# mindazhao/PWStableNet

Measured on AMD Instinct MI355X. Metric: stabilized frames/sec at 256x256 (netG fp32 + grid_sample), whole job, higher is better.
Workload: dtype f32

## Files before the change

### pwstablenet_amd/csrc/conv_common.h

```cpp
#pragma once
#include "common.h"

namespace pws {

typedef float f32x16 __attribute__((ext_vector_type(16)));

struct ConvKParams {
    const float *src_ptr[4];
    int src_c[4];
    int src_ld[4];
    int nsrc;
    int N, H, W;
    int LH, LW;
    int OH, OW;
    int cin_pad;
    int cout;
    const float *w;
    const float *bias;
    float *out;
    int out_ld;
    int act;
    int tiles_x, tiles_y;
    unsigned ntiles;
    int nclasses;
    int cls_inner;
    int ksplit;
    int chunks_per_split;
    size_t split_stride;
    const void *w_bf;
    int kpad_bf, npad_bf;
    int io_bf16;
    int epi16;
    int ndst;
    float *dst_ptr[4];
    int dst_c0[4], dst_c1[4], dst_ld[4], dst_acc[4];
    const void *dst_y[4];
    int dst_y_ld[4], dst_act[4];
    void *out_sign;
    int out_sign_ld;
    const void *dst_sign[4];
    int dst_sign_ld[4];
};

__device__ __forceinline__ void epi_store(const ConvKParams &p, size_t pix, int co, float v) {
    if (p.ndst == 0) {
        p.out[pix * p.out_ld + co] = act_apply(v + (p.bias ? p.bias[co] : 0.f), p.act);
    } else {
#pragma unroll
        for (int s = 0; s < 4; ++s) {
            if (s < p.ndst && co >= p.dst_c0[s] && co < p.dst_c1[s]) {
                float *d = p.dst_ptr[s] + pix * p.dst_ld[s] + (co - p.dst_c0[s]);
                *d = p.dst_acc[s] ? *d + v : v;
            }
        }
    }
}

__device__ __forceinline__ float bf16_lo(unsigned u) { return __builtin_bit_cast(float, u << 16); }
__device__ __forceinline__ float bf16_hi(unsigned u) { return __builtin_bit_cast(float, u & 0xffff0000u); }
__device__ __forceinline__ void epi_store_pair16(const ConvKParams &p, size_t pix, int co, float v0, float v1) {
    if (p.ndst == 0) {
        const float b0 = p.bias ? p.bias[co] : 0.f, b1 = p.bias ? p.bias[co + 1] : 0.f;
        unsigned *d = reinterpret_cast<unsigned *>(reinterpret_cast<__bf16 *>(p.out) + pix * p.out_ld + co);
        *d = cvt_pk_bf16(act_apply(v0 + b0, p.act), act_apply(v1 + b1, p.act));
    } else {
#pragma unroll
        for (int s = 0; s < 4; ++s) {
            if (s < p.ndst && co >= p.dst_c0[s] && co < p.dst_c1[s]) {
                unsigned *d = reinterpret_cast<unsigned *>(reinterpret_cast<__bf16 *>(p.dst_ptr[s]) + pix * p.dst_ld[s] + (co - p.dst_c0[s]));
                if (p.dst_acc[s]) {
                    const unsigned o = *d;
                    v0 += bf16_lo(o), v1 += bf16_hi(o);
                }
                if (p.dst_act[s] != PWS_ACT_NONE) {
                    const unsigned y = *reinterpret_cast<const unsigned *>(static_cast<const __bf16 *>(p.dst_y[s]) + pix * p.dst_y_ld[s] +
                                                                           (co - p.dst_c0[s]));
                    const float sl = p.dst_act[s] == PWS_ACT_LRELU ? 0.2f : 0.f;
                    v0 *= bf16_lo(y) > 0.f ? 1.f : sl, v1 *= bf16_hi(y) > 0.f ? 1.f : sl;
                }
                *d = cvt_pk_bf16(v0, v1);
            }
        }
    }
}

__device__ __forceinline__ void conv_block_coords(const ConvKParams &p, bool subpix, unsigned &tile, int &cls, int &split) {
    if (subpix && p.cls_inner) {
        const unsigned xcd = blockIdx.x & 7u, slot = blockIdx.x >> 3;
        cls = (int)(slot & 3u), split = (int)blockIdx.z;
        tile = xcd_remap(((slot >> 2) << 3) | xcd, p.ntiles);
    } else {
        tile = xcd_remap(blockIdx.x, p.ntiles);
        cls = subpix ? (int)(blockIdx.z & 3) : 0;
        split = subpix ? (int)(blockIdx.z >> 2) : (int)blockIdx.z;
    }
}
static inline dim3 conv_grid(ConvKParams &kp, int bn) {
    kp.cls_inner = kp.nclasses == 4 && kp.ntiles % 8 == 0 ? 1 : 0;
    const unsigned gy = (unsigned)((kp.cout + bn - 1) / bn);
    return kp.cls_inner ? dim3(kp.ntiles * 4, gy, (unsigned)kp.ksplit) : dim3(kp.ntiles, gy, (unsigned)(kp.nclasses * kp.ksplit));
}

struct ProfInfo {
    double flops, bytes;
};

struct TileChoice {
    int th, tw, tn, ck, bn;
    int kid;
    int (*launch)(ConvKParams &, hipStream_t, const ProfInfo &);
};

int launch_splitk_reduce(const ConvKParams &kp, const float *partial, size_t total4, hipStream_t st);

static inline long cdiv(long a, long b) { return (a + b - 1) / b; }

constexpr long kFillBlocks = 512;
constexpr long kFillBlocksBf16 = 256;

[[maybe_unused]] static int select_and_launch(const TileChoice *cands, int ncand, ConvKParams &kp, int cin_total, float *final_out,
                             float *ws, size_t ws_floats, hipStream_t st, const ProfInfo &pi, long kFill = kFillBlocks) {
    const TileChoice *best = nullptr;
    long best_blocks = -1;
    double best_score = -1.0;
// ... 42 lines not shown
```

### pwstablenet_amd/csrc/conv_mfma.hip

```cpp
#include "conv_common.h"

namespace pws {

template <int KS_, int STRIDE_, int PAD_, int SUBPIX_, int TH_, int TW_, int TN_, int CK_, int WM_, int WN_, int MT_,
          int NT_, bool NCHW_ = false>
struct ConvCfg {
    static constexpr int KS = KS_, STRIDE = STRIDE_, PAD = PAD_, TH = TH_, TW = TW_, TN = TN_, CK = CK_;
    static constexpr int SUBPIX = SUBPIX_;
    static constexpr bool CONVT = SUBPIX_ != 0, NCHW = NCHW_;
    static constexpr int WM = WM_, WN = WN_, MT = MT_, NT = NT_;
    static constexpr int THREADS = 64 * WM * WN;
    static constexpr int BM = TH * TW * TN, BN = 32 * NT * WN;
    static_assert(BM == 32 * MT * WM, "tile pixels must equal the M extent of the wave grid");
    static constexpr int IH = (TH - 1) * STRIDE + KS, IW = (TW - 1) * STRIDE + KS;
    static constexpr int PIX = TN * IH * IW;
    static constexpr int CKP = CK + 1;
    static constexpr int TAPS = KS * KS;
    static constexpr int LDS_IN = (PIX * CKP + 3) / 4 * 4;
    static constexpr int LDS_W = TAPS * CK * BN;
    static constexpr int LDS_BYTES = (LDS_IN + LDS_W) * 4;
    static constexpr int C4 = CK / 4;
    static constexpr int ITEMS_IN = (PIX * C4 + THREADS - 1) / THREADS;
    static constexpr int ITEMS_W = (TAPS * CK * (BN / 4) + THREADS - 1) / THREADS;
    static constexpr int ITEMS_NCHW = (PIX * CK + THREADS - 1) / THREADS;
};

template <class C>
__global__ void __launch_bounds__(C::THREADS, 2) conv_mfma_kernel(const ConvKParams p) {
    extern __shared__ float lds[];
    float *lds_in = lds;
    float *lds_w = lds + C::LDS_IN;

    const int tid = threadIdx.x;
    const int lane = tid & 63, wv = tid >> 6;
    const int l31 = lane & 31, hi = lane >> 5;
    const int wm = wv / C::WN, wn = wv % C::WN;

    unsigned tile;
    int cls, split;
    conv_block_coords(p, C::CONVT, tile, cls, split);
    const int tx_i = tile % p.tiles_x;
    const int ty_i = (tile / p.tiles_x) % p.tiles_y;
    const int tn_i = tile / (p.tiles_x * p.tiles_y);
    const int n0 = tn_i * C::TN, y0 = ty_i * C::TH, x0 = tx_i * C::TW;
    const int co0 = blockIdx.y * C::BN;
    const int py = cls >> 1, px = cls & 1;
    const int pad_y = C::SUBPIX == 1 ? 1 - py : (C::SUBPIX == 2 ? 0 : C::PAD);
    const int pad_x = C::SUBPIX == 1 ? 1 - px : (C::SUBPIX == 2 ? 0 : C::PAD);
    const int iy0 = y0 * C::STRIDE - pad_y, ix0 = x0 * C::STRIDE - pad_x;

    int g_pix[C::ITEMS_IN];
    int l_off[C::ITEMS_IN];
    int g_c4[C::ITEMS_IN];
    unsigned ok_mask = 0;
#pragma unroll
    for (int it = 0; it < C::ITEMS_IN; ++it) {
        const int item = tid + it * C::THREADS;
        const int pix = item / C::C4, c4 = item % C::C4;
        const int lx = pix % C::IW, ly = (pix / C::IW) % C::IH, tn = pix / (C::IW * C::IH);
        const int n = n0 + tn, iy = iy0 + ly, ix = ix0 + lx;
        const bool ok = item < C::PIX * C::C4 && n < p.N && iy >= 0 && iy < p.H && ix >= 0 && ix < p.W;
        g_pix[it] = ok ? (n * p.H + iy) * p.W + ix : 0;
        ok_mask |= ok ? (1u << it) : 0u;
        l_off[it] = item < C::PIX * C::C4 ? pix * C::CKP + c4 * 4 : -1;
        g_c4[it] = c4 * 4;
    }
    static_assert(C::ITEMS_IN <= 32 && C::ITEMS_W <= 32, "mask width");
    int w_off[C::ITEMS_W];
    unsigned w_mask = 0;
#pragma unroll
    for (int it = 0; it < C::ITEMS_W; ++it) {
        const int item = tid + it * C::THREADS;
        const int row = item / (C::BN / 4), q = item % (C::BN / 4);
        const int tap = row / C::CK, c = row % C::CK;
        const bool ok = item < C::TAPS * C::CK * (C::BN / 4) && (co0 + q * 4) < p.cout;
        w_off[it] = ok ? (tap * p.cin_pad + c) * p.cout + co0 + q * 4 : 0;
        w_mask |= ok ? (1u << it) : 0u;
    }
    const float *w_cls = p.w + (size_t)cls * C::TAPS * p.cin_pad * p.cout;
    float4 r_in[C::NCHW ? 1 : C::ITEMS_IN];
    float4 r_w[C::ITEMS_W];
    float r_nchw[C::NCHW ? C::ITEMS_NCHW : 1];

    auto load_chunk = [&](int s, int c0, int wrow) {
        if constexpr (C::NCHW) {
            const int Creal = p.src_c[0];
            const size_t sstride = p.src_ld[0] ? (size_t)p.src_ld[0] : (size_t)Creal * p.H * p.W;
#pragma unroll
            for (int it = 0; it < C::ITEMS_NCHW; ++it) {
                const int item = tid + it * C::THREADS;
                const int c = item / C::PIX, pix = item % C::PIX;
                const int lx = pix % C::IW, ly = (pix / C::IW) % C::IH, tn = pix / (C::IW * C::IH);
                const int n = n0 + tn, iy = iy0 + ly, ix = ix0 + lx;
                const bool ok = item < C::PIX * C::CK && (c0 + c) < Creal && n < p.N && iy >= 0 && iy < p.H && ix >= 0 &&
                                ix < p.W;
                const size_t off = ok ? (size_t)n * sstride + ((size_t)(c0 + c) * p.H + iy) * p.W + ix : 0;
                const float v = p.src_ptr[0][off];
                r_nchw[it] = ok ? v : 0.f;
            }
        } else {
            const float *sp = p.src_ptr[s] + c0;
            const size_t ld = p.src_ld[s];
#pragma unroll
            for (int it = 0; it < C::ITEMS_IN; ++it)
                r_in[it] = *reinterpret_cast<const float4 *>(sp + (size_t)g_pix[it] * ld + g_c4[it]);
        }
        const float *wp = w_cls + (size_t)wrow * p.cout;
#pragma unroll
        for (int it = 0; it < C::ITEMS_W; ++it) r_w[it] = *reinterpret_cast<const float4 *>(wp + w_off[it]);
    };
    auto store_chunk = [&]() {
        if constexpr (C::NCHW) {
#pragma unroll
            for (int it = 0; it < C::ITEMS_NCHW; ++it) {
                const int item = tid + it * C::THREADS;
                const int c = item / C::PIX, pix = item % C::PIX;
                if (item < C::PIX * C::CK) lds_in[pix * C::CKP + c] = r_nchw[it];
            }
        } else {
#pragma unroll
            for (int it = 0; it < C::ITEMS_IN; ++it) {
                if (l_off[it] >= 0) {
                    const bool ok = (ok_mask >> it) & 1u;
                    float *d = lds_in + l_off[it];
                    d[0] = ok ? r_in[it].x : 0.f, d[1] = ok ? r_in[it].y : 0.f, d[2] = ok ? r_in[it].z : 0.f,
                    d[3] = ok ? r_in[it].w : 0.f;
                }
            }
        }
#pragma unroll
        for (int it = 0; it < C::ITEMS_W; ++it) {
            const int item = tid + it * C::THREADS;
            if (item < C::TAPS * C::CK * (C::BN / 4)) {
                const bool ok = (w_mask >> it) & 1u;
                *reinterpret_cast<float4 *>(lds_w + item * 4) =
                    ok ? r_w[it] : make_float4(0.f, 0.f, 0.f, 0.f);
            }
        }
    };

    f32x16 acc[C::MT][C::NT];
#pragma unroll
    for (int mt = 0; mt < C::MT; ++mt)
#pragma unroll
        for (int nt = 0; nt < C::NT; ++nt)
#pragma unroll
            for (int r = 0; r < 16; ++r) acc[mt][nt][r] = 0.f;

    int a_base[C::MT];
#pragma unroll
    for (int mt = 0; mt < C::MT; ++mt) {
        const int m = (wm * C::MT + mt) * 32 + l31;
        const int tx = m % C::TW, ty = (m / C::TW) % C::TH, tn = m / (C::TW * C::TH);
        a_base[mt] = ((tn * C::IH + ty * C::STRIDE) * C::IW + tx * C::STRIDE) * C::CKP + hi;
    }
    const int b_base = hi * C::BN + wn * C::NT * 32 + l31;

    int total_chunks = 0;
    if constexpr (C::NCHW) {
        total_chunks = p.cin_pad / C::CK;
    } else {
        for (int s = 0; s < p.nsrc; ++s) total_chunks += p.src_c[s] / C::CK;
    }
    const int ch_begin = split * p.chunks_per_split;
    const int ch_end = min(total_chunks, ch_begin + p.chunks_per_split);
    int s = 0, c0 = ch_begin * C::CK, wrow = ch_begin * C::CK;
    if constexpr (!C::NCHW) {
        while (s < p.nsrc - 1 && c0 >= p.src_c[s]) c0 -= p.src_c[s], ++s;
    }
    if (ch_begin < ch_end) load_chunk(s, c0, wrow);
    for (int ch = ch_begin; ch < ch_end; ++ch) {
        __syncthreads();
        store_chunk();
        __syncthreads();
        c0 += C::CK, wrow += C::CK;
        if (!C::NCHW && c0 >= p.src_c[s]) ++s, c0 = 0;
        if (ch + 1 < ch_end) load_chunk(s, c0, wrow);

#pragma unroll
        for (int tap = 0; tap < C::TAPS; ++tap) {
            if (C::SUBPIX == 2 && ((!py && tap / C::KS) || (!px && tap % C::KS))) continue;
            const int toff = ((tap / C::KS) * C::IW + (tap % C::KS)) * C::CKP;
#pragma unroll
            for (int kk = 0; kk < C::CK / 2; ++kk) {
                float a[C::MT], b[C::NT];
#pragma unroll
                for (int mt = 0; mt < C::MT; ++mt) a[mt] = lds_in[a_base[mt] + toff + 2 * kk];
#pragma unroll
                for (int nt = 0; nt < C::NT; ++nt) b[nt] = lds_w[b_base + (tap * C::CK + 2 * kk) * C::BN + nt * 32];
#pragma unroll
                for (int mt = 0; mt < C::MT; ++mt)
#pragma unroll
                    for (int nt = 0; nt < C::NT; ++nt)
                        acc[mt][nt] = __builtin_amdgcn_mfma_f32_32x32x2f32(a[mt], b[nt], acc[mt][nt], 0, 0, 0);
            }
        }
    }

    const bool partial = p.ksplit > 1;
    float *part = p.out + (size_t)split * p.split_stride;
#pragma unroll
    for (int nt = 0; nt < C::NT; ++nt) {
        const int co = co0 + (wn * C::NT + nt) * 32 + l31;
        const bool co_ok = co < p.cout;
#pragma unroll
        for (int mt = 0; mt < C::MT; ++mt) {
#pragma unroll
            for (int r = 0; r < 16; ++r) {
                const int m = (wm * C::MT + mt) * 32 + (r & 3) + 8 * (r >> 2) + 4 * hi;
                const int tx = m % C::TW, ty = (m / C::TW) % C::TH, tn = m / (C::TW * C::TH);
                const int n = n0 + tn, y = y0 + ty, x = x0 + tx;
                const int oy = C::CONVT ? 2 * y + py : y, ox = C::CONVT ? 2 * x + px : x;
                if (co_ok && n < p.N && y < p.LH && x < p.LW && oy < p.OH && ox < p.OW) {
                    const size_t pix = (size_t)(n * p.OH + oy) * p.OW + ox;
                    if (partial)
                        part[pix * p.cout + co] = acc[mt][nt][r];
                    else
                        epi_store(p, pix, co, acc[mt][nt][r]);
                }
            }
        }
    }
}

__global__ void __launch_bounds__(256) splitk_reduce_kernel(const ConvKParams p, const float *__restrict__ partial,
                                                            size_t total4) {
    const size_t i = (size_t)blockIdx.x * 256 + threadIdx.x;
    if (i >= total4) return;
    float4 a = reinterpret_cast<const float4 *>(partial)[i];
    for (int s = 1; s < p.ksplit; ++s) {
        const float4 b = reinterpret_cast<const float4 *>(partial + (size_t)s * p.split_stride)[i];
        a.x += b.x, a.y += b.y, a.z += b.z, a.w += b.w;
    }
    const size_t pix = (i * 4) / p.cout;
    const int co = (int)((i * 4) % p.cout);
    if (p.io_bf16) {
        epi_store_pair16(p, pix, co, a.x, a.y), epi_store_pair16(p, pix, co + 2, a.z, a.w);
        return;
    }
    epi_store(p, pix, co, a.x), epi_store(p, pix, co + 1, a.y), epi_store(p, pix, co + 2, a.z), epi_store(p, pix, co + 3, a.w);
}

int launch_splitk_reduce(const ConvKParams &kp, const float *partial, size_t total4, hipStream_t st) {
    hipLaunchKernelGGL(splitk_reduce_kernel, dim3((unsigned)((total4 + 255) / 256)), dim3(256), 0, st, kp, partial, total4);
    return check_launch("splitk_reduce_kernel");
}

template <class C, int KID>
static int launch_cfg(ConvKParams &kp, hipStream_t st, const ProfInfo &pi) {
    static PerDeviceFlag attr_set_dev;
    bool &attr_set = attr_set_dev.cur();
    if (!attr_set) {
        hipError_t e = hipFuncSetAttribute(reinterpret_cast<const void *>(&conv_mfma_kernel<C>),
                                           hipFuncAttributeMaxDynamicSharedMemorySize, C::LDS_BYTES);
        if (e != hipSuccess) {
            set_error("hipFuncSetAttribute(conv_mfma_kernel, %d B LDS): %s", C::LDS_BYTES, hipGetErrorString(e));
            return PWS_EHIP;
        }
        attr_set = true;
    }
    const dim3 grid = conv_grid(kp, C::BN);
    hipLaunchKernelGGL(conv_mfma_kernel<C>, grid, dim3(C::THREADS), C::LDS_BYTES, st, kp);
    return check_launch("conv_mfma_kernel");
}

template <class C, int KID>
static constexpr TileChoice choice() {
    return TileChoice{C::TH, C::TW, C::TN, C::CK, C::BN, KID, &launch_cfg<C, KID>};
}

using K3S1_T256 = ConvCfg<3, 1, 1, 0, 16, 16, 1, 16, 4, 1, 2, 2>;
using K3S1_T128 = ConvCfg<3, 1, 1, 0, 8, 16, 1, 16, 4, 1, 1, 2>;
using K3S1_T64 = ConvCfg<3, 1, 1, 0, 8, 8, 1, 16, 2, 2, 1, 1>;
using K3S1_T64N4 = ConvCfg<3, 1, 1, 0, 4, 4, 4, 16, 2, 2, 1, 1>;
using K3S1_T64N16 = ConvCfg<3, 1, 1, 0, 2, 2, 16, 16, 2, 2, 1, 1>;
using K3S2_T256 = ConvCfg<3, 2, 1, 0, 16, 16, 1, 8, 4, 1, 2, 2>;
using K3S2_T128 = ConvCfg<3, 2, 1, 0, 8, 16, 1, 16, 4, 1, 1, 2>;
using K3S2_T64 = ConvCfg<3, 2, 1, 0, 8, 8, 1, 16, 2, 2, 1, 1>;
using K3S2_T64N4 = ConvCfg<3, 2, 1, 0, 4, 4, 4, 16, 2, 2, 1, 1>;
using K3S2_T64N16 = ConvCfg<3, 2, 1, 0, 2, 2, 16, 16, 2, 2, 1, 1>;
using K5S1_T256 = ConvCfg<5, 1, 2, 0, 16, 16, 1, 8, 4, 1, 2, 2>;
using K5S1_T256_NCHW = ConvCfg<5, 1, 2, 0, 16, 16, 1, 8, 4, 1, 2, 2, true>;
using CT4_T256 = ConvCfg<2, 1, 0, 1, 16, 16, 1, 16, 4, 1, 2, 2>;
using CT4_T128 = ConvCfg<2, 1, 0, 1, 8, 16, 1, 16, 4, 1, 1, 2>;
using CT4_T64 = ConvCfg<2, 1, 0, 1, 8, 8, 1, 16, 2, 2, 1, 1>;
using CT4_T64N4 = ConvCfg<2, 1, 0, 1, 4, 4, 4, 16, 2, 2, 1, 1>;
using CT4_T64N16 = ConvCfg<2, 1, 0, 1, 2, 2, 16, 16, 2, 2, 1, 1>;

using K4S2_T256 = ConvCfg<4, 2, 1, 0, 16, 16, 1, 8, 4, 1, 2, 2>;
using K4S2_T128 = ConvCfg<4, 2, 1, 0, 8, 16, 1, 8, 4, 1, 1, 2>;
using K4S2_T64 = ConvCfg<4, 2, 1, 0, 8, 8, 1, 8, 2, 2, 1, 1>;
using K4S2_T64N4 = ConvCfg<4, 2, 1, 0, 4, 4, 4, 8, 2, 2, 1, 1>;
using K4S2_T64N16 = ConvCfg<4, 2, 1, 0, 2, 2, 16, 8, 2, 2, 1, 1>;
using SP3_T256 = ConvCfg<2, 1, 0, 2, 16, 16, 1, 16, 4, 1, 2, 2>;
using SP3_T128 = ConvCfg<2, 1, 0, 2, 8, 16, 1, 16, 4, 1, 1, 2>;
using SP3_T64 = ConvCfg<2, 1, 0, 2, 8, 8, 1, 16, 2, 2, 1, 1>;
using SP3_T64N4 = ConvCfg<2, 1, 0, 2, 4, 4, 4, 16, 2, 2, 1, 1>;
using SP3_T64N16 = ConvCfg<2, 1, 0, 2, 2, 2, 16, 16, 2, 2, 1, 1>;

static const TileChoice kK3S1[] = {choice<K3S1_T256, KID_CONV_K3S1_BIG>(), choice<K3S1_T128, KID_CONV_K3S1_BIG>(),
                                   choice<K3S1_T64, KID_CONV_K3S1_SMALL>(), choice<K3S1_T64N4, KID_CONV_K3S1_SMALL>(),
                                   choice<K3S1_T64N16, KID_CONV_K3S1_SMALL>()};
static const TileChoice kK3S2[] = {choice<K3S2_T256, KID_CONV_K3S2_BIG>(), choice<K3S2_T128, KID_CONV_K3S2_BIG>(),
                                   choice<K3S2_T64, KID_CONV_K3S2_SMALL>(), choice<K3S2_T64N4, KID_CONV_K3S2_SMALL>(),
                                   choice<K3S2_T64N16, KID_CONV_K3S2_SMALL>()};
static const TileChoice kCT4[] = {choice<CT4_T256, KID_CONVT4_BIG>(), choice<CT4_T128, KID_CONVT4_BIG>(),
                                  choice<CT4_T64, KID_CONVT4_SMALL>(), choice<CT4_T64N4, KID_CONVT4_SMALL>(),
                                  choice<CT4_T64N16, KID_CONVT4_SMALL>()};
static const TileChoice kK4S2[] = {choice<K4S2_T256, KID_DGRAD_K4S2>(), choice<K4S2_T128, KID_DGRAD_K4S2>(),
                                   choice<K4S2_T64, KID_DGRAD_K4S2>(), choice<K4S2_T64N4, KID_DGRAD_K4S2>(),
                                   choice<K4S2_T64N16, KID_DGRAD_K4S2>()};
static const TileChoice kSP3[] = {choice<SP3_T256, KID_DGRAD_SP3>(), choice<SP3_T128, KID_DGRAD_SP3>(),
                                  choice<SP3_T64, KID_DGRAD_SP3>(), choice<SP3_T64N4, KID_DGRAD_SP3>(),
                                  choice<SP3_T64N16, KID_DGRAD_SP3>()};
static const TileChoice kK5[] = {choice<K5S1_T256, KID_CONV_K5S1>()};
static const TileChoice kK5N[] = {choice<K5S1_T256_NCHW, KID_CONV_K5S1>()};

int conv_bf16_fwd(int kind, ConvKParams &kp, int cin_total, float *out, float *ws, size_t ws_floats, hipStream_t st,
                  const ProfInfo &pi);
int conv_bf16_dgrad(int kind, ConvKParams &kp, int cout_f, float *ws, size_t ws_floats, hipStream_t st, const ProfInfo &pi);
static inline bool ledger_direct(int bit) { return (exp_mask(EXP_PARITY_LEDGER, 32) & bit) != 0; }
int conv_ringf_try(int kind, const ConvKParams &kp, hipStream_t st, const ProfInfo &pi);
int conv_first_try(const ConvKParams &kp, hipStream_t st, const ProfInfo &pi);
int wino5_first_try(const ConvKParams &kp, const float *u, hipStream_t st, const ProfInfo &pi);
int conv_skinny_try(int kind, ConvKParams &kp, float *final_out, float *ws, size_t ws_floats, hipStream_t st, const ProfInfo &pi);

int conv2d_fwd_impl(const pws_conv_args *a, hipStream_t st) {
    PWS_REQUIRE(a != nullptr, "pws_conv2d_fwd: args is NULL");
    PWS_REQUIRE(a->n >= 0 && a->h > 0 && a->w > 0, "pws_conv2d_fwd: bad n/h/w %d/%d/%d", a->n, a->h, a->w);
    PWS_REQUIRE(a->nsrc >= 1 && a->nsrc <= 4, "pws_conv2d_fwd: nsrc %d not in 1..4", a->nsrc);
    PWS_REQUIRE(a->cout > 0 && a->cout % 4 == 0, "pws_conv2d_fwd: cout %d must be a positive multiple of 4", a->cout);
    PWS_REQUIRE(a->out && a->w_packed, "pws_conv2d_fwd: NULL out / w_packed");
    PWS_REQUIRE(a->out_ld >= a->cout, "pws_conv2d_fwd: out_ld %d < cout %d", a->out_ld, a->cout);
    PWS_REQUIRE(a->act >= PWS_ACT_NONE && a->act <= PWS_ACT_RELU, "pws_conv2d_fwd: bad act %d", a->act);
    PWS_REQUIRE(a->ws == nullptr || (reinterpret_cast<size_t>(a->ws) & 15) == 0, "pws_conv2d_fwd: ws must be 16-B aligned");
    if (a->n == 0) return PWS_OK;

    ConvKParams kp{};
    int cin = 0;
    kp.nsrc = a->nsrc;
    const bool nchw = a->src_nchw != 0;
    if (nchw) {
        PWS_REQUIRE(a->kind == PWS_CONV_K5S1 && a->nsrc == 1, "pws_conv2d_fwd: NCHW source only for the k5 first layer");
        PWS_REQUIRE(a->src[0].ptr && a->src[0].channels > 0, "pws_conv2d_fwd: bad NCHW source");
        PWS_REQUIRE(a->src[0].ld >= 0, "pws_conv2d_fwd: NCHW source: ld is the sample stride in floats (0 = dense)");
        kp.src_ptr[0] = a->src[0].ptr, kp.src_c[0] = a->src[0].channels, kp.src_ld[0] = a->src[0].ld;
        cin = a->src[0].channels;
    } else {
        for (int s = 0; s < a->nsrc; ++s) {
            const pws_src &sr = a->src[s];
            PWS_REQUIRE(sr.ptr && sr.channels > 0 && sr.channels % 16 == 0 && sr.ld >= sr.channels && sr.ld % 4 == 0 &&
                            (reinterpret_cast<size_t>(sr.ptr) & 15) == 0,
                        "pws_conv2d_fwd: source %d (channels %d, ld %d) must be 16-B aligned, channels %% 16 == 0, ld %% 4 == 0",
                        s, sr.channels, sr.ld);
            kp.src_ptr[s] = sr.ptr, kp.src_c[s] = sr.channels, kp.src_ld[s] = sr.ld;
            cin += sr.channels;
        }
    }
    kp.cin_pad = (cin + 15) / 16 * 16;
    kp.N = a->n, kp.H = a->h, kp.W = a->w;
    kp.cout = a->cout, kp.w = a->w_packed, kp.bias = a->bias, kp.out_ld = a->out_ld, kp.act = a->act;
    kp.nclasses = 1;
    PWS_REQUIRE((size_t)a->n * a->h * a->w < (1u << 31), "pws_conv2d_fwd: n*h*w too large for 32-bit pixel indices");
    float *ws = static_cast<float *>(a->ws);
    const size_t ws_floats = a->ws_bytes / sizeof(float);
    const bool bf16 = a->math == PWS_MATH_BF16 && a->w_bf16 && !nchw;
    if (a->store == PWS_STORE_BF16) {
        PWS_REQUIRE(bf16, "pws_conv2d_fwd: bf16 storage needs math == PWS_MATH_BF16, w_bf16 and NHWC sources");
        PWS_REQUIRE(a->out_ld % 2 == 0 && a->cout % 2 == 0 && (reinterpret_cast<size_t>(a->out) & 3) == 0,
                    "pws_conv2d_fwd: bf16 storage needs an even cout / out_ld and a 4-byte aligned out");
        for (int s = 0; s < a->nsrc; ++s)
            PWS_REQUIRE(a->src[s].channels % 32 == 0 && a->src[s].ld % 8 == 0,
                        "pws_conv2d_fwd: bf16 storage needs channels %% 32 == 0 and ld %% 8 == 0 (source %d: %d, %d)", s,
                        a->src[s].channels, a->src[s].ld);
        kp.io_bf16 = 1;
        kp.epi16 = a->cout % 8 == 0 && a->out_ld % 8 == 0 && (reinterpret_cast<size_t>(a->out) & 15) == 0;
    }
    kp.w_bf = a->w_bf16, kp.kpad_bf = (kp.cin_pad + 31) / 32 * 32, kp.npad_bf = (a->cout + 63) / 64 * 64;
    if (a->out_sign) {
        PWS_REQUIRE(a->store == PWS_STORE_BF16 && a->cout % 8 == 0 && a->out_sign_ld >= a->cout / 8,
                    "pws_conv2d_fwd: out_sign needs bf16 storage, cout %% 8 == 0 and out_sign_ld >= cout / 8");
        kp.out_sign = a->out_sign, kp.out_sign_ld = a->out_sign_ld;
    }

    auto info = [&](int k2, double out_pix) {
        ProfInfo pi;
        pi.flops = 2.0 * out_pix * a->cout * (double)cin * k2;
        const double es = a->store == PWS_STORE_BF16 ? 2.0 : 4.0, ws_ = bf16 ? 2.0 : 4.0;
        pi.bytes = es * ((double)a->n * a->h * a->w * cin + out_pix * a->cout) + ws_ * (double)k2 * cin * a->cout;
        return pi;
    };
// ... 180 lines not shown
```

### pwstablenet_amd/csrc/experiments.h

```cpp
#pragma once

namespace pws {

extern int g_experiment;

enum Exp : int {
    EXP_GS_BWD_GENERAL = 2,
    EXP_U8_CVT_SHIFT = 4,
    EXP_GS_ROWWIN = 5,
    EXP_NO_SIGN_BITS = 12,
    EXP_NETG_PER_STAGE = 15,
    EXP_RING_OFF = 20,
    EXP_RING_SMALL = 21,
    EXP_RINGF_OFF = 22,
    EXP_RINGF_8X32 = 23,
    EXP_RINGF_16X32 = 24,
    EXP_FIRST_MFMA = 25,
    EXP_FIRST_NO_WINO = 26,
    EXP_RINGF_32CH = 27,
    EXP_FIRST_SMALL = 29,
    EXP_WINO5_SMALL = 30,
    EXP_HEAD_V1 = 35,
    EXP_GS_U8_LANE_WINDOWS = 49,
    EXP_WRING_OFF = 50,
    EXP_WRING_FORCE = 58,
    EXP_WRING_MODE2 = 59,
    EXP_SKINNY_OFF = 70,
    EXP_SKINNY16_OFF = 71,
    EXP_SKINNY16_4096 = 72,
    EXP_SKINNY_SKIP = 73,
    EXP_WGRAD_RING_OFF = 80,
    EXP_WGRAD_RING_FORCE = 81,
    EXP_HEAD_VALU = 90,
    EXP_HEAD_BWD_VALU = 91,
    EXP_HEAD_ONE_TILE = 92,
    EXP_DEEP_TILE_ALWAYS = 96,
    EXP_SHAPE_GENERAL = 97,
    EXP_TL1_TILED = 98,
    EXP_RING_8WAVE = 105,
    EXP_SMOOTH_ONE_PIXEL = 110,
    EXP_NO_PACK_ONE_PASS = 120,
    EXP_RING_UNIT256 = 186,
    EXP_RING_UNIT128 = 187,
    EXP_WGRAD_NO_MERGE = 188,
    EXP_WGRAD_MIN_TILES = 190,
    EXP_FIRST_ABLATE = 1100,
    EXP_FIRST_CLOCK = 1200,
    EXP_WINO5_ABLATE = 1300,
    EXP_WGRAD_WIDE_ABLATE = 1400,
    EXP_RING_ABLATE = 1500,
    EXP_WINO_ABLATE = 1600,
    EXP_BF16_PROBE = 2100,
    EXP_RINGF_VARIANT = 2200,
    EXP_PARITY_LEDGER = 3000,
    EXP_WRING_ABLATE = 4000,
};

inline bool exp_is(Exp e) { return g_experiment == e; }
inline bool exp_in(Exp base, int n) { return g_experiment >= base && g_experiment < base + n; }
inline int exp_mask(Exp base, int n) { return exp_in(base, n) ? g_experiment - base : 0; }

}
```

### pwstablenet_amd/hipabi.py

```python
import contextlib
import ctypes
import os

_HERE = os.path.dirname(os.path.abspath(__file__))
LIB_PATH = os.environ.get("PWS_LIB_PATH") or os.path.join(_HERE, "libpwstable_hip.so")

c_f32p = ctypes.c_void_p
c_stream = ctypes.c_void_p

ACT_NONE, ACT_LRELU, ACT_RELU = 0, 1, 2
OPT_TWO_QUEUES = 1
OPT_MATH, MATH_FP32, MATH_BF16 = 2, 0, 1
OPT_STORE, STORE_FP32, STORE_BF16 = 3, 0, 1
ABI_VERSION = 5
NETG_DETERMINISTIC = 1
NETG_PRUNE_DEAD = 2
OPT_EXPERIMENT = 100


class Exp:
    GS_BWD_GENERAL = 2
    U8_CVT_SHIFT = 4
    GS_ROWWIN = 5
    NO_SIGN_BITS = 12
    NETG_PER_STAGE = 15
    RING_OFF = 20
    RING_SMALL = 21
    RINGF_OFF = 22
    RINGF_8X32 = 23
    RINGF_16X32 = 24
    FIRST_MFMA = 25
    FIRST_NO_WINO = 26
    RINGF_32CH = 27
    FIRST_SMALL = 29
    WINO5_SMALL = 30
    HEAD_V1 = 35
    GS_U8_LANE_WINDOWS = 49
    WRING_OFF = 50
    WRING_FORCE = 58
    WRING_MODE2 = 59
    SKINNY_OFF = 70
    SKINNY16_OFF = 71
    SKINNY16_4096 = 72
    SKINNY_SKIP = 73
    WGRAD_RING_OFF = 80
    WGRAD_RING_FORCE = 81
    HEAD_VALU = 90
    HEAD_BWD_VALU = 91
    HEAD_ONE_TILE = 92
    DEEP_TILE_ALWAYS = 96
    SHAPE_GENERAL = 97
    TL1_TILED = 98
    RING_8WAVE = 105
    SMOOTH_ONE_PIXEL = 110
    NO_PACK_ONE_PASS = 120
    RING_UNIT256 = 186
    RING_UNIT128 = 187
    WGRAD_NO_MERGE = 188
    WGRAD_MIN_TILES = 190
    FIRST_ABLATE = 1100
    FIRST_CLOCK = 1200
    WINO5_ABLATE = 1300
    WGRAD_WIDE_ABLATE = 1400
    RING_ABLATE = 1500
    WINO_ABLATE = 1600
    BF16_PROBE = 2100
    RINGF_VARIANT = 2200
    PARITY_LEDGER = 3000
    WRING_ABLATE = 4000
OBJ_SLOTS = 64
CONV_K3S1, CONV_K3S2, CONV_K5S1, CONVT_K3S1, CONVT_K4S2, CONV_K2S1P0, CONV_K1, CONV_K3S1_OUT = range(8)


class PwsSrc(ctypes.Structure):
    _fields_ = [("ptr", ctypes.c_void_p), ("channels", ctypes.c_int), ("ld", ctypes.c_int)]


class PwsConvArgs(ctypes.Structure):
    _fields_ = [("kind", ctypes.c_int), ("n", ctypes.c_int), ("h", ctypes.c_int), ("w", ctypes.c_int),
                ("nsrc", ctypes.c_int), ("src", PwsSrc * 4), ("src_nchw", ctypes.c_int), ("cout", ctypes.c_int),
                ("w_packed", ctypes.c_void_p), ("bias", ctypes.c_void_p), ("act", ctypes.c_int),
                ("out", ctypes.c_void_p), ("out_ld", ctypes.c_int), ("w_wino", ctypes.c_void_p), ("ws", ctypes.c_void_p),
                ("ws_bytes", ctypes.c_size_t), ("math", ctypes.c_int), ("w_bf16", ctypes.c_void_p), ("store", ctypes.c_int),
                ("w_wring", ctypes.c_void_p), ("out_sign", ctypes.c_void_p), ("out_sign_ld", ctypes.c_int)]


class PwsDst(ctypes.Structure):
    _fields_ = [("ptr", ctypes.c_void_p), ("channels", ctypes.c_int), ("ld", ctypes.c_int), ("accumulate", ctypes.c_int),
                ("act_y", ctypes.c_void_p), ("act_y_ld", ctypes.c_int), ("act", ctypes.c_int),
                ("act_sign", ctypes.c_void_p), ("act_sign_ld", ctypes.c_int)]


class PwsConvBwdDataArgs(ctypes.Structure):
    _fields_ = [("kind", ctypes.c_int), ("n", ctypes.c_int), ("h", ctypes.c_int), ("w", ctypes.c_int), ("cout", ctypes.c_int),
                ("gout", ctypes.c_void_p), ("gout_ld", ctypes.c_int), ("w_dgrad", ctypes.c_void_p), ("ndst", ctypes.c_int),
                ("dst", PwsDst * 4), ("ws", ctypes.c_void_p), ("ws_bytes", ctypes.c_size_t), ("math", ctypes.c_int),
                ("w_dgrad_bf16", ctypes.c_void_p), ("store", ctypes.c_int)]


class PwsConvBwdWeightArgs(ctypes.Structure):
    _fields_ = [("kind", ctypes.c_int), ("n", ctypes.c_int), ("h", ctypes.c_int), ("w", ctypes.c_int), ("nsrc", ctypes.c_int),
                ("src", PwsSrc * 4), ("src_nchw", ctypes.c_int), ("cout", ctypes.c_int), ("gout", ctypes.c_void_p),
                ("gout_ld", ctypes.c_int), ("dw_packed", ctypes.c_void_p), ("math", ctypes.c_int), ("store", ctypes.c_int),
                ("dbias", ctypes.c_void_p), ("deterministic", ctypes.c_int), ("src2_ptr", ctypes.c_void_p * 4), ("gout2", ctypes.c_void_p)]


class PwsNetgOpts(ctypes.Structure):
    _fields_ = [("math", ctypes.c_int), ("store", ctypes.c_int), ("two_queues", ctypes.c_int), ("flags", ctypes.c_int),
                ("x_sample_stride", ctypes.c_size_t)]


class PwsProfRecord(ctypes.Structure):
    _fields_ = [("kernel_id", ctypes.c_int), ("tag", ctypes.c_int), ("flops", ctypes.c_double),
                ("bytes", ctypes.c_double), ("ms", ctypes.c_float)]


_I, _S, _P = ctypes.c_int, ctypes.c_size_t, ctypes.c_void_p
_F = ctypes.c_float
SIGNATURES = {
    "pws_version": (_I, []),
    "pws_last_error": (ctypes.c_char_p, []),
    "pws_set_option": (_I, [_I, _I]),
    "pws_get_option": (_I, [_I]),
    "pws_packed_bf16_floats": (_S, [_I, _I, _I]),
    "pws_pack_weight_bf16": (_I, [_P, _P, _I, _I, _I, _P]),
    "pws_nchw_to_nhwc_pad": (_I, [_P, _P, _I, _I, _I, _I, _I, _P]),
    "pws_nchw_to_nhwc_pad_s": (_I, [_P, _P, _I, _I, _I, _I, _I, _I, _P]),
    "pws_cvt_bf16_to_f32": (_I, [_P, _P, _S, _P]),
    "pws_cvt_f32_to_bf16": (_I, [_P, _P, _S, _I, _P]),
    "pws_device_info": (_I, [ctypes.POINTER(_I), ctypes.POINTER(_I)]),
    "pws_packed_weight_floats": (_S, [_I, _I, _I]),
    "pws_pack_conv_weight": (_I, [_P, _P, _I, _I, _I, _P]),
    "pws_packed_wino_floats": (_S, [_I, _I]),
    "pws_pack_conv_weight_wino": (_I, [_P, _P, _I, _I, _P]),
    "pws_packed_wring_floats": (_S, [_I, _I, _I]),
    "pws_pack_conv_weight_wring": (_I, [_P, _P, _I, _I, _I, _P]),
    "pws_packed_wino_ct4_floats": (_S, [_I, _I]),
    "pws_pack_conv_weight_wino_ct4": (_I, [_P, _P, _I, _I, _P]),
    "pws_conv2d_fwd": (_I, [ctypes.POINTER(PwsConvArgs), _P]),
    "pws_act_bwd_bias": (_I, [_P, _P, _S, _I, _I, _P, _P]),
    "pws_act_bwd_bias_s": (_I, [_P, _P, _S, _I, _I, _P, _I, _P, _S, _P]),
    "pws_act_bwd_bias_ws_bytes": (_S, [_I]),
    "pws_packed_dgrad_floats": (_S, [_I, _I, _I]),
    "pws_pack_conv_weight_dgrad": (_I, [_P, _P, _I, _I, _I, _P]),
    "pws_conv2d_bwd_data": (_I, [ctypes.POINTER(PwsConvBwdDataArgs), _P]),
    "pws_conv2d_bwd_weight": (_I, [ctypes.POINTER(PwsConvBwdWeightArgs), _P]),
    "pws_unpack_conv_weight": (_I, [_P, _P, _I, _I, _I, _P]),
    "pws_theta_head_fwd_save": (_I, [_P, _I, _I, _I, _P, _P, _P, _P, _P, _P, _P, _P]),
# ... 186 lines not shown
```

Baseline: 2026.

## Add buffer-load, tap-pipelined variant of small-tile MFMA conv kernel

Adds a GEN=2 variant of the MFMA conv kernel for the small-tile configs (K3S1, K3S2, ConvT4). It uses raw buffer loads with out-of-bounds offsets in place of masked global loads, and redirects padded LDS writes to a dummy slot so stores need no branch. It also double-buffers per-tap LDS-to-register reads so the next tap's operands load while the current tap's MFMAs run. The variant is the default whenever the 32-bit offsets fit; experiment flags can force the old path or ablate stages. The cost is higher register pressure and more template instantiations.

New measurement: 2027 (median of 3 runs). About the same (+0.1%).

```diff
diff --git a/pwstablenet_amd/csrc/conv_common.h b/pwstablenet_amd/csrc/conv_common.h
--- a/pwstablenet_amd/csrc/conv_common.h
+++ b/pwstablenet_amd/csrc/conv_common.h
@@ -40,6 +40,7 @@
     int out_sign_ld;
     const void *dst_sign[4];
     int dst_sign_ld[4];
+    int ablate;
 };
 
 __device__ __forceinline__ void epi_store(const ConvKParams &p, size_t pix, int co, float v) {
diff --git a/pwstablenet_amd/csrc/conv_mfma.hip b/pwstablenet_amd/csrc/conv_mfma.hip
--- a/pwstablenet_amd/csrc/conv_mfma.hip
+++ b/pwstablenet_amd/csrc/conv_mfma.hip
@@ -19,15 +19,17 @@
     static constexpr int LDS_IN = (PIX * CKP + 3) / 4 * 4;
     static constexpr int LDS_W = TAPS * CK * BN;
     static constexpr int LDS_BYTES = (LDS_IN + LDS_W) * 4;
+    static constexpr int LDS_BYTES_G2 = LDS_BYTES + 16;
     static constexpr int C4 = CK / 4;
     static constexpr int ITEMS_IN = (PIX * C4 + THREADS - 1) / THREADS;
     static constexpr int ITEMS_W = (TAPS * CK * (BN / 4) + THREADS - 1) / THREADS;
     static constexpr int ITEMS_NCHW = (PIX * CK + THREADS - 1) / THREADS;
 };
 
-template <class C>
+template <class C, int GEN>
 __global__ void __launch_bounds__(C::THREADS, 2) conv_mfma_kernel(const ConvKParams p) {
     extern __shared__ float lds[];
+    const int abl = GEN ? p.ablate : 0;
     float *lds_in = lds;
     float *lds_w = lds + C::LDS_IN;
 
@@ -78,11 +80,40 @@
         w_mask |= ok ? (1u << it) : 0u;
     }
     const float *w_cls = p.w + (size_t)cls * C::TAPS * p.cin_pad * p.cout;
+    constexpr unsigned kOob = 0x80000000u, kRecords = 0x7fffffffu;
+    unsigned v_in[GEN == 2 ? C::ITEMS_IN : 1], v_w[GEN == 2 ? C::ITEMS_W : 1];
+    auto set_src = [&](int sn) {
+        if constexpr (GEN == 2) {
+            const int ld = p.src_ld[sn];
+#pragma unroll
+            for (int it = 0; it < C::ITEMS_IN; ++it)
+                v_in[it] = (ok_mask >> it) & 1u ? (unsigned)(g_pix[it] * ld + g_c4[it]) * 4u : kOob;
+        }
+    };
+    if constexpr (GEN == 2) {
+        static_assert(!C::NCHW, "NHWC sources only");
+#pragma unroll
+        for (int it = 0; it < C::ITEMS_W; ++it) v_w[it] = (w_mask >> it) & 1u ? (unsigned)w_off[it] * 4u : kOob;
+#pragma unroll
+        for (int it = 0; it < C::ITEMS_IN; ++it)
+            if (l_off[it] < 0) l_off[it] = C::LDS_IN + C::LDS_W;
+    }
     float4 r_in[C::NCHW ? 1 : C::ITEMS_IN];
     float4 r_w[C::ITEMS_W];
     float r_nchw[C::NCHW ? C::ITEMS_NCHW : 1];
 
     auto load_chunk = [&](int s, int c0, int wrow) {
+        if constexpr (GEN == 2) {
+            const __amdgpu_buffer_rsrc_t rs = __builtin_amdgcn_make_buffer_rsrc(const_cast<float *>(p.src_ptr[s]), 0, (int)kRecords, 0x00020000);
+#pragma unroll
+            for (int it = 0; it < C::ITEMS_IN; ++it)
+                r_in[it] = __builtin_bit_cast(float4, __builtin_amdgcn_raw_buffer_load_b128(rs, (int)v_in[it], c0 * 4, 0));
+            const __amdgpu_buffer_rsrc_t rw = __builtin_amdgcn_make_buffer_rsrc(const_cast<float *>(w_cls), 0, (int)kRecords, 0x00020000);
+#pragma unroll
+            for (int it = 0; it < C::ITEMS_W; ++it)
+                r_w[it] = __builtin_bit_cast(float4, __builtin_amdgcn_raw_buffer_load_b128(rw, (int)v_w[it], wrow * p.cout * 4, 0));
+            return;
+        }
         if constexpr (C::NCHW) {
             const int Creal = p.src_c[0];
             const size_t sstride = p.src_ld[0] ? (size_t)p.src_ld[0] : (size_t)Creal * p.H * p.W;
@@ -110,6 +141,19 @@
         for (int it = 0; it < C::ITEMS_W; ++it) r_w[it] = *reinterpret_cast<const float4 *>(wp + w_off[it]);
     };
     auto store_chunk = [&]() {
+        if constexpr (GEN == 2) {
+#pragma unroll
+            for (int it = 0; it < C::ITEMS_IN; ++it) {
+                float *d = lds_in + l_off[it];
+                d[0] = r_in[it].x, d[1] = r_in[it].y, d[2] = r_in[it].z, d[3] = r_in[it].w;
+            }
+#pragma unroll
+            for (int it = 0; it < C::ITEMS_W; ++it) {
+                const int item = tid + it * C::THREADS;
+                if (item < C::TAPS * C::CK * (C::BN / 4)) *reinterpret_cast<float4 *>(lds_w + item * 4) = r_w[it];
+            }
+            return;
+        }
         if constexpr (C::NCHW) {
 #pragma unroll
             for (int it = 0; it < C::ITEMS_NCHW; ++it) {
@@ -168,14 +212,53 @@
     if constexpr (!C::NCHW) {
         while (s < p.nsrc - 1 && c0 >= p.src_c[s]) c0 -= p.src_c[s], ++s;
     }
+    set_src(s);
     if (ch_begin < ch_end) load_chunk(s, c0, wrow);
     for (int ch = ch_begin; ch < ch_end; ++ch) {
-        __syncthreads();
-        store_chunk();
-        __syncthreads();
+        if (!(abl & 8)) __syncthreads();
+        if (!(abl & 4)) store_chunk();
+        if (!(abl & 8)) __syncthreads();
         c0 += C::CK, wrow += C::CK;
-        if (!C::NCHW && c0 >= p.src_c[s]) ++s, c0 = 0;
-        if (ch + 1 < ch_end) load_chunk(s, c0, wrow);
+        if (!C::NCHW && c0 >= p.src_c[s]) {
+            ++s, c0 = 0;
+            if (s < p.nsrc) set_src(s);
+        }
+        if (ch + 1 < ch_end && !(abl & 2)) load_chunk(s, c0, wrow);
+        if (abl & 1) continue;
+
+        if constexpr (GEN == 2) {
+            static_assert(C::SUBPIX != 2, "no tap is skipped in the pipelined walk");
+            float a[2][C::MT][C::CK / 2], b[2][C::NT][C::CK / 2];
+            auto read_tap = [&](int tap, float (&ta)[C::MT][C::CK / 2], float (&tb)[C::NT][C::CK / 2]) {
+                const int toff = ((tap / C::KS) * C::IW + (tap % C::KS)) * C::CKP;
+#pragma unroll
+                for (int kk = 0; kk < C::CK / 2; ++kk) {
+#pragma unroll
+                    for (int mt = 0; mt < C::MT; ++mt) ta[mt][kk] = lds_in[a_base[mt] + toff + 2 * kk];
+#pragma unroll
+                    for (int nt = 0; nt < C::NT; ++nt) tb[nt][kk] = lds_w[b_base + (tap * C::CK + 2 * kk) * C::BN + nt * 32];
+                }
+            };
+            read_tap(0, a[0], b[0]);
+#pragma unroll
+            for (int tap = 0; tap < C::TAPS; ++tap) {
+#pragma unroll
+                for (int kk = 0; kk < C::CK / 2; ++kk) {
+                    if (kk == 1 && tap + 1 < C::TAPS) {
+                        __builtin_amdgcn_sched_barrier(0);
+                        read_tap(tap + 1, a[(tap + 1) & 1], b[(tap + 1) & 1]);
+                        __builtin_amdgcn_sched_barrier(0);
+                    }
+#pragma unroll
+                    for (int mt = 0; mt < C::MT; ++mt)
+#pragma unroll
+                        for (int nt = 0; nt < C::NT; ++nt)
+                            acc[mt][nt] = __builtin_amdgcn_mfma_f32_32x32x2f32(a[tap & 1][mt][kk], b[tap & 1][nt][kk], acc[mt][nt], 0, 0, 0);
+                }
+                __builtin_amdgcn_sched_barrier(0);
+            }
+            continue;
+        }
 
 #pragma unroll
         for (int tap = 0; tap < C::TAPS; ++tap) {
@@ -246,27 +329,40 @@
     return check_launch("splitk_reduce_kernel");
 }
 
-template <class C, int KID>
+template <class C, int KID, int GEN = 0>
 static int launch_cfg(ConvKParams &kp, hipStream_t st, const ProfInfo &pi) {
     static PerDeviceFlag attr_set_dev;
     bool &attr_set = attr_set_dev.cur();
     if (!attr_set) {
-        hipError_t e = hipFuncSetAttribute(reinterpret_cast<const void *>(&conv_mfma_kernel<C>),
-                                           hipFuncAttributeMaxDynamicSharedMemorySize, C::LDS_BYTES);
+        hipError_t e = hipFuncSetAttribute(reinterpret_cast<const void *>(&conv_mfma_kernel<C, GEN>),
+                                           hipFuncAttributeMaxDynamicSharedMemorySize, GEN == 2 ? C::LDS_BYTES_G2 : C::LDS_BYTES);
         if (e != hipSuccess) {
-            set_error("hipFuncSetAttribute(conv_mfma_kernel, %d B LDS): %s", C::LDS_BYTES, hipGetErrorString(e));
+            set_error("hipFuncSetAttribute(conv_mfma_kernel, %d B LDS): %s", GEN == 2 ? C::LDS_BYTES_G2 : C::LDS_BYTES, hipGetErrorString(e));
             return PWS_EHIP;
         }
         attr_set = true;
     }
     const dim3 grid = conv_grid(kp, C::BN);
-    hipLaunchKernelGGL(conv_mfma_kernel<C>, grid, dim3(C::THREADS), C::LDS_BYTES, st, kp);
+    hipLaunchKernelGGL((conv_mfma_kernel<C, GEN>), grid, dim3(C::THREADS), GEN == 2 ? C::LDS_BYTES_G2 : C::LDS_BYTES, st, kp);
     return check_launch("conv_mfma_kernel");
 }
 
 template <class C, int KID>
 static constexpr TileChoice choice() {
     return TileChoice{C::TH, C::TW, C::TN, C::CK, C::BN, KID, &launch_cfg<C, KID>};
+}
+
+template <class C, int KID>
+static int launch_small(ConvKParams &kp, hipStream_t st, const ProfInfo &pi) {
+    const int m = exp_mask(EXP_CONV_ABLATE, 32), v = m >> 4;
+    kp.ablate = m & 15;
+    bool fits = (size_t)kp.nclasses * C::TAPS * kp.cin_pad * kp.cout * 4 < (1u << 31);
+    for (int s = 0; s < kp.nsrc; ++s) fits = fits && (size_t)kp.N * kp.H * kp.W * kp.src_ld[s] * 4 < (1u << 31);
+    return exp_is(EXP_CONV_SMALL_V1) || v == 1 || !fits ? launch_cfg<C, KID, 1>(kp, st, pi) : launch_cfg<C, KID, 2>(kp, st, pi);
+}
+template <class C, int KID>
+static constexpr TileChoice small_choice() {
+    return TileChoice{C::TH, C::TW, C::TN, C::CK, C::BN, KID, &launch_small<C, KID>};
 }
 
 using K3S1_T256 = ConvCfg<3, 1, 1, 0, 16, 16, 1, 16, 4, 1, 2, 2>;
@@ -299,14 +395,14 @@
 using SP3_T64N16 = ConvCfg<2, 1, 0, 2, 2, 2, 16, 16, 2, 2, 1, 1>;
 
 static const TileChoice kK3S1[] = {choice<K3S1_T256, KID_CONV_K3S1_BIG>(), choice<K3S1_T128, KID_CONV_K3S1_BIG>(),
-                                   choice<K3S1_T64, KID_CONV_K3S1_SMALL>(), choice<K3S1_T64N4, KID_CONV_K3S1_SMALL>(),
-                                   choice<K3S1_T64N16, KID_CONV_K3S1_SMALL>()};
+                                   small_choice<K3S1_T64, KID_CONV_K3S1_SMALL>(), small_choice<K3S1_T64N4, KID_CONV_K3S1_SMALL>(),
+                                   small_choice<K3S1_T64N16, KID_CONV_K3S1_SMALL>()};
 static const TileChoice kK3S2[] = {choice<K3S2_T256, KID_CONV_K3S2_BIG>(), choice<K3S2_T128, KID_CONV_K3S2_BIG>(),
-                                   choice<K3S2_T64, KID_CONV_K3S2_SMALL>(), choice<K3S2_T64N4, KID_CONV_K3S2_SMALL>(),
-                                   choice<K3S2_T64N16, KID_CONV_K3S2_SMALL>()};
+                                   small_choice<K3S2_T64, KID_CONV_K3S2_SMALL>(), small_choice<K3S2_T64N4, KID_CONV_K3S2_SMALL>(),
+                                   small_choice<K3S2_T64N16, KID_CONV_K3S2_SMALL>()};
 static const TileChoice kCT4[] = {choice<CT4_T256, KID_CONVT4_BIG>(), choice<CT4_T128, KID_CONVT4_BIG>(),
-                                  choice<CT4_T64, KID_CONVT4_SMALL>(), choice<CT4_T64N4, KID_CONVT4_SMALL>(),
-                                  choice<CT4_T64N16, KID_CONVT4_SMALL>()};
+                                  small_choice<CT4_T64, KID_CONVT4_SMALL>(), small_choice<CT4_T64N4, KID_CONVT4_SMALL>(),
+                                  small_choice<CT4_T64N16, KID_CONVT4_SMALL>()};
 static const TileChoice kK4S2[] = {choice<K4S2_T256, KID_DGRAD_K4S2>(), choice<K4S2_T128, KID_DGRAD_K4S2>(),
                                    choice<K4S2_T64, KID_DGRAD_K4S2>(), choice<K4S2_T64N4, KID_DGRAD_K4S2>(),
                                    choice<K4S2_T64N16, KID_DGRAD_K4S2>()};
diff --git a/pwstablenet_amd/csrc/experiments.h b/pwstablenet_amd/csrc/experiments.h
--- a/pwstablenet_amd/csrc/experiments.h
+++ b/pwstablenet_amd/csrc/experiments.h
@@ -34,6 +34,7 @@
     EXP_HEAD_VALU = 90,
     EXP_HEAD_BWD_VALU = 91,
     EXP_HEAD_ONE_TILE = 92,
+    EXP_CONV_SMALL_V1 = 95,
     EXP_DEEP_TILE_ALWAYS = 96,
     EXP_SHAPE_GENERAL = 97,
     EXP_TL1_TILED = 98,
@@ -50,6 +51,7 @@
     EXP_WGRAD_WIDE_ABLATE = 1400,
     EXP_RING_ABLATE = 1500,
     EXP_WINO_ABLATE = 1600,
+    EXP_CONV_ABLATE = 1700,
     EXP_BF16_PROBE = 2100,
     EXP_RINGF_VARIANT = 2200,
     EXP_PARITY_LEDGER = 3000,
diff --git a/pwstablenet_amd/hipabi.py b/pwstablenet_amd/hipabi.py
--- a/pwstablenet_amd/hipabi.py
+++ b/pwstablenet_amd/hipabi.py
@@ -48,6 +48,7 @@
     HEAD_VALU = 90
     HEAD_BWD_VALU = 91
     HEAD_ONE_TILE = 92
+    CONV_SMALL_V1 = 95
     DEEP_TILE_ALWAYS = 96
     SHAPE_GENERAL = 97
     TL1_TILED = 98
@@ -64,6 +65,7 @@
     WGRAD_WIDE_ABLATE = 1400
     RING_ABLATE = 1500
     WINO_ABLATE = 1600
+    CONV_ABLATE = 1700
     BF16_PROBE = 2100
     RINGF_VARIANT = 2200
     PARITY_LEDGER = 3000
```
